# breuner/elbencho

Hardware: AMD Instinct MI355X
Metric: seq-read GiB/s into GPU HBM (higher is better)
Workload: dtype raw-bytes; 1 GPU; seqread; model=storage-benchmark seq-read into HBM, threads_per_gpu=16, block_size=4194304, iodepth=1, bench_dir=/dev/shm/elbencho_amd_bench, gpu_staged=True, mmap_zero_copy=True, dynamic_slice=True, verify_on_gpu=True, verify_salt=7, parallelism=single, device=AMD Radeon Graphics, device_numa_node=1

## Files before the change

elbencho_amd/csrc/engine.cpp:

```cpp

#include "engine.h"

#include <fcntl.h>
#include <linux/fs.h>
#include <pthread.h>
#include <sched.h>
#include <sys/ioctl.h>
#include <sys/mman.h>
#include <sys/stat.h>
#include <sys/types.h>
#include <unistd.h>

#include <algorithm>
#include <random>
#include <cerrno>
#include <cstdio>
#include <cstring>

#include "netbench.h"
#include "uring.h"

namespace eb {

static constexpr uint64_t INTERRUPT_CHECK_INTERVAL = 128;
// ... 477 lines not shown

    if (gpu && (fileOff % 8 == 0) && (len % 16 == 0)) {
        GpuVerifyResult r = gpu->verifyChecksumDev(slot, len, fileOff, (uint64_t)cfg.verifySalt);
        if (r.numMismatches)
            throw WorkerError("Data verification failed (GPU). First bad file offset: " +
                              std::to_string(r.firstBadFileOffset) +
                              "; mismatching 8-byte words: " + std::to_string(r.numMismatches));
        return;
    }

    uint64_t bad = verifyChecksumCPU(hostBufs[slot], len, fileOff, (uint64_t)cfg.verifySalt);
    if (bad != UINT64_MAX)
        throw WorkerError("Data verification failed. First bad file offset: " +
                          std::to_string(bad));
}


namespace {

struct FdGuard {
    std::vector<int> fds;
    ~FdGuard()
    {
        for (int fd : fds)
            if (fd >= 0) close(fd);
    }
};

struct MmapGuard {
    std::vector<std::pair<char*, uint64_t>> maps;

    void map(int fd, uint64_t len, bool writable, int madvFlags, const std::string& path)
    {
        int prot = writable ? (PROT_READ | PROT_WRITE) : PROT_READ;
        void* p = mmap(nullptr, len, prot, MAP_SHARED, fd, 0);
        if (p == MAP_FAILED)
            throw WorkerError("mmap failed. Path: " + path + "; SysErr: " + strerror(errno));
        if (madvFlags && madvise(p, len, madvFlags))
            throw WorkerError("madvise failed. Path: " + path);
        maps.emplace_back((char*)p, len);
    }

    char* base(uint64_t idx) const
    {
        return idx < maps.size() ? maps[idx].first : nullptr;
    }

    ~MmapGuard()
    {
        for (auto& [p, len] : maps) munmap(p, len);
    }
};

enum FadvBits {
    FADV_BIT_SEQ = 1,
    FADV_BIT_RAND = 2,
    FADV_BIT_WILLNEED = 4,
    FADV_BIT_DONTNEED = 8,
    FADV_BIT_NOREUSE = 16,
};

inline void applyFadvise(int fd, int bits, const std::string& path)
{
    if (!bits) return;
    struct { int bit; int advice; } table[] = {
        {FADV_BIT_SEQ, POSIX_FADV_SEQUENTIAL},   {FADV_BIT_RAND, POSIX_FADV_RANDOM},
        {FADV_BIT_WILLNEED, POSIX_FADV_WILLNEED}, {FADV_BIT_DONTNEED, POSIX_FADV_DONTNEED},
        {FADV_BIT_NOREUSE, POSIX_FADV_NOREUSE},
    };
    for (auto& e : table)
        if ((bits & e.bit) && posix_fadvise(fd, 0, 0, e.advice))
            throw WorkerError("posix_fadvise failed. Path: " + path);
}

}

void Worker::fileModeBlocks(bool isWrite)
{
    const auto& cfg = eng.cfg;
    if (cfg.ioDepth > 1) return fileModeBlocksUring(isWrite);
    if (cfg.useMmap && !cfg.gpuIDs.empty() && cfg.flockMode == 0 &&
        !(isWrite && (cfg.rwMixPct > 0 || cfg.rwMixThreads > 0)) && !cfg.verifyDirect &&
        cfg.pathType == PathType::FILE && !eng.opsLog.isEnabled())
        return fileModeBlocksGpuMmap(isWrite);

    const uint64_t fileSize = eng.effFileSize;
    const uint64_t bs = cfg.blockSize;
    const size_t numFiles = cfg.paths.size();
    const uint64_t numBlocksPerFile = (fileSize + bs - 1) / bs;
    const bool rwMixActive = isWrite && (cfg.rwMixPct > 0 || isDedicatedReader);

    FdGuard fg;
    MmapGuard mg;
    int rwFlags = isWrite
                      ? ((cfg.verifyDirect || rwMixActive || cfg.useMmap) ? O_RDWR : O_WRONLY)
                      : O_RDONLY;
    int openFlags = rwFlags | (cfg.directIO ? O_DIRECT : 0);
    if (isWrite && cfg.pathType == PathType::FILE) openFlags |= O_CREAT;
    for (const auto& p : cfg.paths) {
        int fd = open(p.c_str(), openFlags, 0644);
        if (fd < 0) throwErrno("open", p);
        fg.fds.push_back(fd);
        if (isWrite && cfg.pathType == PathType::FILE) {
            if (cfg.truncate && ftruncate(fd, 0)) throwErrno("truncate", p);
            if ((cfg.truncToSize != UINT64_MAX || cfg.useMmap) && ftruncate(fd, fileSize))
                throwErrno("truncate-to-size", p);
            if (cfg.preallocFile && fallocate(fd, 0, 0, fileSize)) throwErrno("fallocate", p);
        }
        applyFadvise(fd, cfg.fadviseFlags, p);
        if (cfg.useMmap) mg.map(fd, fileSize, isWrite, cfg.madviseFlags, p);
    }

    const uint64_t mapBPF = (cfg.random || cfg.strided) ? (fileSize / bs) : numBlocksPerFile;
    const uint64_t virtFileLen = mapBPF * bs;

    auto mapBlock = [&](const BlockSpec& s, uint64_t& fileIdx, uint64_t& inFileOff,
                        uint64_t& ioLen) -> bool {
        if (!virtFileLen) return false;
        fileIdx = s.offset / virtFileLen;
        if (fileIdx >= numFiles) return false;
        inFileOff = s.offset - fileIdx * virtFileLen;
        if (inFileOff >= fileSize) return false;
        ioLen = std::min(s.len, fileSize - inFileOff);
        return true;
    };

    std::unique_ptr<OffsetGen> gen;
    if (cfg.random || cfg.strided) {
        uint64_t numBlocksTotal = mapBPF * numFiles;
        uint64_t rangeLen = bs * (numBlocksTotal / cfg.numDataSetThreads);
        uint64_t rangeOff = (uint64_t)globalRank * rangeLen;
        if (cfg.strided) {
            gen = std::make_unique<OffsetGenStrided>(bs, globalRank, cfg.numDataSetThreads);
            gen->reset(0, bs * numBlocksTotal);
        } else {
            gen = makeOffsetGen(rangeOff, rangeLen);
        }
    } else {
        uint64_t myStart, myLen;
        fairShareSlice(virtFileLen * numFiles, myStart, myLen);
        if (!myLen) return;
        gen = makeOffsetGen(myStart, myLen);
    }

    static const bool pipelineDisabled = [] {
        const char* v = getenv("EB_GPU_PIPELINE");
        return v && v[0] == '0';
    }();
    const bool gpuPipelined = gpu && !pipelineDisabled && cfg.ioDepth == 1 &&
                              !cfg.useMmap && cfg.flockMode == 0 &&
                              !rwMixActive && !cfg.verifyDirect && hostBufs.size() >= 2 &&
                              !eng.opsLog.isEnabled();
    if (gpuPipelined) {
        constexpr uint64_t VERIFY_FETCH_INTERVAL = 64;
        const bool doVerify = cfg.verifySalt >= 0;
        const bool lat = cfg.measureLat;
        const int nSlots = (int)hostBufs.size();
        std::vector<char> slotBusy(nSlots, 0);
        uint64_t sinceFetch = 0;
        BlockSpec spec;
        uint64_t opCount = 0;

        auto fetchVerify = [&]() {
            GpuVerifyResult r = gpu->fetchVerifyResult();
            if (r.numMismatches)
                throw WorkerError(
                    "Data verification failed (GPU). First bad file offset: " +
                    std::to_string(r.firstBadFileOffset) + "; mismatching 8-byte words: " +
                    std::to_string(r.numMismatches));
        };

        if (isWrite) {
            int slot = 0;
            bool havePrev = false;
            int prevSlot = 0;
            uint64_t prevFileIdx = 0, prevInFileOff = 0, prevIoLen = 0;

            for (;;) {
                bool haveCur = false;
                uint64_t fileIdx = 0, inFileOff = 0, ioLen = 0;
                while (gen->next(spec)) {
                    if (mapBlock(spec, fileIdx, inFileOff, ioLen)) {
                        haveCur = true;
                        break;
                    }
                }

                if (haveCur) {
                    if ((opCount++ % INTERRUPT_CHECK_INTERVAL) == 0) checkInterrupt();
                    rateLimiter.wait(ioLen);
                    if (slotBusy[slot]) gpu->waitSlotEvent(slot);
                    preWriteFill(slot, ioLen, inFileOff);
                    if (lat) gpu->recordTimedStart(slot);
                    gpu->copyD2HAsync(slot, ioLen);
                    if (lat) gpu->recordTimedEnd(slot);
                    gpu->recordSlotEvent(slot);
                    slotBusy[slot] = 1;
                }

                if (havePrev) {
                    gpu->waitSlotEvent(prevSlot);
                    uint64_t copyUs = (lat && gpu->timedPairActive(prevSlot))
                                          ? gpu->timedElapsedUSec(prevSlot) : 0;
                    auto t0 = lat ? Clock::now() : Clock::time_point();
                    ssize_t res = pwrite(fg.fds[prevFileIdx], hostBufs[prevSlot],
                                         prevIoLen, prevInFileOff);
                    if (res != (ssize_t)prevIoLen) throwErrno("write", cfg.paths[prevFileIdx]);
                    if (lat)
                        addIoLat(copyUs + (uint64_t)std::chrono::duration_cast<
                            std::chrono::microseconds>(Clock::now() - t0).count());
                    liveOps.bytes.fetch_add(prevIoLen, std::memory_order_relaxed);
                    liveOps.iops.fetch_add(1, std::memory_order_relaxed);
                }

                if (!haveCur) break;
                havePrev = true;
                prevSlot = slot;
                prevFileIdx = fileIdx;
                prevInFileOff = inFileOff;
                prevIoLen = ioLen;
                slot = (slot + 1) % nSlots;
            }
            if (cfg.fsyncPerFile)
                for (size_t i = 0; i < fg.fds.size(); i++)
                    if (fsync(fg.fds[i])) throwErrno("fsync", cfg.paths[i]);
        } else if (!doVerify && gpuBatchSlots(cfg.blockSize) >= 2 && nSlots >= 4) {
            const int batch = gpuBatchSlots(cfg.blockSize);
            int half = 0;
            bool halfBusy[2] = {false, false};
            std::vector<uint64_t> blkUs[2];
            int halfCount[2] = {0, 0};
            if (lat) {
                blkUs[0].resize(batch);
                blkUs[1].resize(batch);
            }

            auto collectHalfLat = [&](int h) {
                if (!lat || !halfCount[h]) return;
                int b = h * batch;
                if (!gpu->timedPairActive(b)) return;
                uint64_t share = gpu->timedElapsedUSec(b) / (uint64_t)halfCount[h];
                for (int i = 0; i < halfCount[h]; i++)
                    addIoLat(blkUs[h][i] + share);
                halfCount[h] = 0;
            };

            int filled = 0;
            int base = 0;
            while (gen->next(spec)) {
                uint64_t fileIdx, inFileOff, ioLen;
                if (!mapBlock(spec, fileIdx, inFileOff, ioLen)) continue;

                if (filled == 0) {
                    if ((opCount++ % 4) == 0) checkInterrupt();
                    base = half * batch;
                    if (halfBusy[half]) {
                        gpu->waitSlotEvent(base);
                        collectHalfLat(half);
                    }
                }

                rateLimiter.wait(ioLen);
                auto t0 = lat ? Clock::now() : Clock::time_point();
                ssize_t res = pread(fg.fds[fileIdx], hostBufs[base + filled], ioLen,
                                    inFileOff);
                if (res != (ssize_t)ioLen) throwErrno("read", cfg.paths[fileIdx]);
                if (lat)
                    blkUs[half][filled] = (uint64_t)std::chrono::duration_cast<
                        std::chrono::microseconds>(Clock::now() - t0).count();
                liveOps.bytes.fetch_add(ioLen, std::memory_order_relaxed);
                liveOps.iops.fetch_add(1, std::memory_order_relaxed);
                filled++;

                if (filled == batch) {
                    if (lat) {
                        halfCount[half] = batch;
                        gpu->recordTimedStart(base);
                    }
                    gpu->copyH2DRangeAsync(base, batch);
                    if (lat) gpu->recordTimedEnd(base);
                    gpu->recordSlotEvent(base);
                    halfBusy[half] = true;
                    half ^= 1;
                    filled = 0;
                }
            }
            if (filled) {
                int b = half * batch;
                if (lat) {
                    halfCount[half] = filled;
                    gpu->recordTimedStart(b);
                }
                gpu->copyH2DRangeAsync(b, filled);
                if (lat) gpu->recordTimedEnd(b);
            }
            if (lat) {
                gpu->syncStream();
                collectHalfLat(0);
                collectHalfLat(1);
            }
        } else {
            int slot = 0;
            std::vector<uint64_t> preadUs(lat ? nSlots : 0, 0);
            while (gen->next(spec)) {
                if ((opCount++ % INTERRUPT_CHECK_INTERVAL) == 0) checkInterrupt();

                uint64_t fileIdx, inFileOff, ioLen;
                if (!mapBlock(spec, fileIdx, inFileOff, ioLen)) continue;

                rateLimiter.wait(ioLen);
                if (slotBusy[slot]) gpu->waitSlotEvent(slot);
                if (lat && gpu->timedPairActive(slot))
                    addIoLat(preadUs[slot] + gpu->timedElapsedUSec(slot));

                auto t0 = lat ? Clock::now() : Clock::time_point();
                ssize_t res = pread(fg.fds[fileIdx], hostBufs[slot], ioLen, inFileOff);
                if (res != (ssize_t)ioLen) throwErrno("read", cfg.paths[fileIdx]);
                if (lat) {
                    preadUs[slot] = (uint64_t)std::chrono::duration_cast<
                        std::chrono::microseconds>(Clock::now() - t0).count();
                    gpu->recordTimedStart(slot);
                }

                gpu->copyH2DAsync(slot, ioLen);
                if (lat) gpu->recordTimedEnd(slot);
                if (doVerify) {
                    if ((inFileOff % 8 == 0) && (ioLen % 16 == 0)) {
                        gpu->verifyChecksumDevAsync(slot, ioLen, inFileOff,
                                                    (uint64_t)cfg.verifySalt);
                        if (++sinceFetch >= VERIFY_FETCH_INTERVAL) {
                            fetchVerify();
                            sinceFetch = 0;
                        }
                    } else {
                        uint64_t bad = verifyChecksumCPU(hostBufs[slot], ioLen, inFileOff,
                                                         (uint64_t)cfg.verifySalt);
                        if (bad != UINT64_MAX)
                            throw WorkerError(
                                "Data verification failed. First bad file offset: " +
                                std::to_string(bad));
                    }
                }
                gpu->recordSlotEvent(slot);
                slotBusy[slot] = 1;

                liveOps.bytes.fetch_add(ioLen, std::memory_order_relaxed);
                liveOps.iops.fetch_add(1, std::memory_order_relaxed);
                slot = (slot + 1) % nSlots;
            }
            if (doVerify) fetchVerify();
            if (lat) {
                gpu->syncStream();
                for (int s = 0; s < nSlots; s++)
                    if (gpu->timedPairActive(s))
                        addIoLat(preadUs[s] + gpu->timedElapsedUSec(s));
            }
        }

        gpu->syncStream();
        return;
    }

    const bool lat = cfg.measureLat;
    BlockSpec spec;
    uint64_t opCount = 0;

    while (gen->next(spec)) {
        if ((opCount++ % INTERRUPT_CHECK_INTERVAL) == 0) checkInterrupt();

        uint64_t fileIdx, inFileOff, ioLen;
        if (!mapBlock(spec, fileIdx, inFileOff, ioLen)) continue;

        bool mixRead = rwMixActive &&
                       (isDedicatedReader ||
                        (cfg.rwMixThreads == 0 && rwMixDecideRead()));
        bool blockWrite = isWrite && !mixRead;

        if (rwMixActive && rwBalancerActive()) rwBalanceWait(mixRead, ioLen);

        auto t0 = lat ? Clock::now() : Clock::time_point();

        ssize_t res = blockIO(blockWrite, fg.fds[fileIdx], 0, ioLen, inFileOff,
                              mg.base(fileIdx), &cfg.paths[fileIdx]);
        if (res < 0)
            throwErrno(blockWrite ? "write" : "read", cfg.paths[fileIdx]);
        if ((uint64_t)res != ioLen)
            throw WorkerError(std::string("unexpected short ") + (blockWrite ? "write" : "read") +
                              ". Path: " + cfg.paths[fileIdx] +
                              "; expected: " + std::to_string(ioLen) +
                              "; got: " + std::to_string(res) +
                              (mixRead ? "; Hint: rwmix reads need a pre-written file." : ""));

        if (lat)
            addIoLat((uint64_t)std::chrono::duration_cast<std::chrono::microseconds>(
                Clock::now() - t0).count(), mixRead);

        AtomicLiveOps& ops = mixRead ? liveOpsReadMix : liveOps;
        ops.bytes.fetch_add(ioLen, std::memory_order_relaxed);
        ops.iops.fetch_add(1, std::memory_order_relaxed);
        if (rwMixActive && rwBalancerActive()) rwBalanceAccount(mixRead, ioLen);
    }

    if (isWrite && cfg.fsyncPerFile)
        for (size_t i = 0; i < fg.fds.size(); i++)
            if (fsync(fg.fds[i])) throwErrno("fsync", cfg.paths[i]);
}

void Worker::fileModeBlocksGpuMmap(bool isWrite)
{
    const auto& cfg = eng.cfg;
    const uint64_t fileSize = eng.effFileSize;
    const uint64_t bs = cfg.blockSize;
    const size_t numFiles = cfg.paths.size();
    const uint64_t numBlocksPerFile = (fileSize + bs - 1) / bs;
    const bool doVerify = cfg.verifySalt >= 0;
    const bool lat = cfg.measureLat;

    std::vector<char*> bases(numFiles);
    for (size_t i = 0; i < numFiles; i++)
        bases[i] = eng.getMappedReg(cfg.paths[i], fileSize, isWrite).base;

    const uint64_t mapBPF = (cfg.random || cfg.strided) ? (fileSize / bs) : numBlocksPerFile;
    const uint64_t virtFileLen = mapBPF * bs;

    const bool dynamic = cfg.dynamicSlice && !cfg.random && !cfg.strided &&
                         !cfg.backward && cfg.numThreads == cfg.numDataSetThreads;

    std::unique_ptr<OffsetGen> gen;
    if (dynamic) {
    } else if (cfg.random || cfg.strided) {
        uint64_t numBlocksTotal = mapBPF * numFiles;
        uint64_t rangeLen = bs * (numBlocksTotal / cfg.numDataSetThreads);
        uint64_t rangeOff = (uint64_t)globalRank * rangeLen;
        if (cfg.strided) {
            gen = std::make_unique<OffsetGenStrided>(bs, globalRank, cfg.numDataSetThreads);
            gen->reset(0, bs * numBlocksTotal);
        } else {
            gen = makeOffsetGen(rangeOff, rangeLen);
        }
    } else {
        uint64_t myStart, myLen;
        fairShareSlice(virtFileLen * numFiles, myStart, myLen);
        if (!myLen) return;
        gen = makeOffsetGen(myStart, myLen);
    }

    const int nSlots = (int)hostBufs.size();
    constexpr uint64_t VERIFY_FETCH_INTERVAL = 64;
    uint64_t sinceFetch = 0;
    BlockSpec spec;
    uint64_t opCount = 0;
    int slot = 0;

    auto fetchVerify = [&]() {
        GpuVerifyResult r = gpu->fetchVerifyResult();
        if (r.numMismatches)
            throw WorkerError("Data verification failed (GPU). First bad file offset: " +
                              std::to_string(r.firstBadFileOffset) +
                              "; mismatching 8-byte words: " +
                              std::to_string(r.numMismatches));
    };

    const uint64_t totalBlocks = numBlocksPerFile * numFiles;

    auto nextBlock = [&](uint64_t& fileIdx, uint64_t& inFileOff,
                         uint64_t& ioLen) -> bool {
        if (dynamic) {
            for (;;) {
                uint64_t b = eng.dynCursor.fetch_add(1, std::memory_order_relaxed);
                if (b >= totalBlocks) return false;
                fileIdx = b / numBlocksPerFile;
                inFileOff = (b % numBlocksPerFile) * bs;
                if (inFileOff >= fileSize) continue;
                ioLen = std::min(bs, fileSize - inFileOff);
                return true;
            }
        }
        while (gen->next(spec)) {
            if (!virtFileLen) return false;
            fileIdx = spec.offset / virtFileLen;
            if (fileIdx >= numFiles) continue;
            inFileOff = spec.offset - fileIdx * virtFileLen;
            if (inFileOff >= fileSize) continue;
            ioLen = std::min(spec.len, fileSize - inFileOff);
            return true;
        }
        return false;
    };

    uint64_t fileIdx, inFileOff, ioLen;
    while (nextBlock(fileIdx, inFileOff, ioLen)) {
        if ((opCount++ % INTERRUPT_CHECK_INTERVAL) == 0) checkInterrupt();

        rateLimiter.wait(ioLen);

        if (lat && gpu->timedPairActive(slot))
            addIoLat(gpu->timedElapsedUSec(slot));

        if (isWrite) {
            preWriteFill(slot, ioLen, inFileOff);
            if (lat) gpu->recordTimedStart(slot);
            gpu->copyToHostAsync(slot, bases[fileIdx] + inFileOff, ioLen);
            if (lat) gpu->recordTimedEnd(slot);
        } else {
            if (lat) gpu->recordTimedStart(slot);
            gpu->copyFromHostAsync(slot, bases[fileIdx] + inFileOff, ioLen);
            if (lat) gpu->recordTimedEnd(slot);
            if (doVerify && (inFileOff % 8 == 0) && (ioLen % 16 == 0)) {
                gpu->verifyChecksumDevAsync(slot, ioLen, inFileOff,
                                            (uint64_t)cfg.verifySalt);
                if (++sinceFetch >= VERIFY_FETCH_INTERVAL) {
                    fetchVerify();
                    sinceFetch = 0;
                }
            } else if (doVerify) {
                uint64_t bad = verifyChecksumCPU(bases[fileIdx] + inFileOff, ioLen,
                                                 inFileOff, (uint64_t)cfg.verifySalt);
                if (bad != UINT64_MAX)
                    throw WorkerError("Data verification failed. First bad file offset: " +
                                      std::to_string(bad));
            }
        }

        liveOps.bytes.fetch_add(ioLen, std::memory_order_relaxed);
        liveOps.iops.fetch_add(1, std::memory_order_relaxed);
        slot = (slot + 1) % nSlots;

        if ((opCount & 127) == 0) gpu->syncStream();
    }

    gpu->syncStream();
    if (lat)
        for (int s = 0; s < nSlots; s++)
            if (gpu->timedPairActive(s)) addIoLat(gpu->timedElapsedUSec(s));
    if (doVerify && !isWrite) fetchVerify();
}

void Worker::fileModeBlocksUring(bool isWrite)
{
    const auto& cfg = eng.cfg;
    const uint64_t fileSize = eng.effFileSize;
    const uint64_t bs = cfg.blockSize;
    const size_t numFiles = cfg.paths.size();
    const uint64_t numBlocksPerFile = (fileSize + bs - 1) / bs;
    const int depth = cfg.ioDepth;
    const bool lat = cfg.measureLat;

    const bool rwMixActive = isWrite && (cfg.rwMixPct > 0 || isDedicatedReader);

    FdGuard fg;
    int rwFlags = isWrite ? ((cfg.verifyDirect || rwMixActive) ? O_RDWR : O_WRONLY) : O_RDONLY;
    int openFlags = rwFlags | (cfg.directIO ? O_DIRECT : 0);
    if (isWrite && cfg.pathType == PathType::FILE) openFlags |= O_CREAT;
    for (const auto& p : cfg.paths) {
        int fd = open(p.c_str(), openFlags, 0644);
        if (fd < 0) throwErrno("open", p);
        fg.fds.push_back(fd);
        if (isWrite && cfg.pathType == PathType::FILE) {
            if (cfg.truncate && ftruncate(fd, 0)) throwErrno("truncate", p);
            if (cfg.truncToSize != UINT64_MAX && ftruncate(fd, fileSize))
                throwErrno("truncate-to-size", p);
            if (cfg.preallocFile && fallocate(fd, 0, 0, fileSize)) throwErrno("fallocate", p);
        }
        applyFadvise(fd, cfg.fadviseFlags, p);
    }

    const uint64_t mapBPF = (cfg.random || cfg.strided) ? (fileSize / bs) : numBlocksPerFile;
    const uint64_t virtFileLen = mapBPF * bs;

    auto mapBlock = [&](const BlockSpec& s, uint64_t& fileIdx, uint64_t& inFileOff,
                        uint64_t& ioLen) -> bool {
        if (!virtFileLen) return false;
        fileIdx = s.offset / virtFileLen;
        if (fileIdx >= numFiles) return false;
        inFileOff = s.offset - fileIdx * virtFileLen;
        if (inFileOff >= fileSize) return false;
        ioLen = std::min(s.len, fileSize - inFileOff);
        return true;
    };

    std::unique_ptr<OffsetGen> gen;
    if (cfg.random || cfg.strided) {
        uint64_t numBlocksTotal = mapBPF * numFiles;
        uint64_t rangeLen = bs * (numBlocksTotal / cfg.numDataSetThreads);
        uint64_t rangeOff = (uint64_t)globalRank * rangeLen;
        if (cfg.strided) {
            gen = std::make_unique<OffsetGenStrided>(bs, globalRank, cfg.numDataSetThreads);
            gen->reset(0, bs * numBlocksTotal);
        } else {
            gen = makeOffsetGen(rangeOff, rangeLen);
        }
    } else {
        uint64_t myStart, myLen;
        fairShareSlice(virtFileLen * numFiles, myStart, myLen);
        if (!myLen) return;
        gen = makeOffsetGen(myStart, myLen);
    }

    IoUring ring;
    ring.init(depth);

    if (!getenv("EB_URING_NOFIXED")) {
        std::vector<struct iovec> iovs(depth);
        for (int s = 0; s < depth; s++)
            iovs[s] = {hostBufs[s], (size_t)bs};
        ring.registerBuffers(iovs.data(), depth);
        ring.registerFiles(fg.fds.data(), (unsigned)fg.fds.size());
    }

    const int gpuBatch = gpu ? gpuBatchSlots(bs) : 1;
    const bool batchedRead = gpu && !isWrite && cfg.verifySalt < 0 &&
                             gpuBatch >= 2 && depth >= 4 &&
                             getenv("EB_GPU_URING_BATCH");
    if (getenv("EB_DEBUG_PATH"))
        fprintf(stderr, "[eb] uring path: gpu=%d batchedRead=%d batch=%d depth=%d\n",
                gpu ? 1 : 0, (int)batchedRead, gpuBatch, depth);
    if (batchedRead) {
        const int halfSize = std::min(depth / 2, 64);
        struct Op {
            uint64_t off = 0, len = 0;
            Clock::time_point start;
            int fileIdx = 0;
        };
        std::vector<Op> ops(2 * halfSize);
        std::vector<IoUring::Completion> bcomps(depth);
        int submitted[2] = {0, 0}, done[2] = {0, 0};
        bool exhausted2 = false;
        BlockSpec bspec;

        auto fillHalf = [&](int h) -> int {
            int base = h * halfSize;
            int n = 0;
            while (n < halfSize && !exhausted2) {
                uint64_t fileIdx = 0, inFileOff = 0, ioLen = 0;
                for (;;) {
                    if (!gen->next(bspec)) { exhausted2 = true; break; }
                    if (mapBlock(bspec, fileIdx, inFileOff, ioLen)) break;
                }
                if (exhausted2) break;
                rateLimiter.wait(ioLen);
                int slot = base + n;
                ops[slot] = {inFileOff, ioLen,
                             lat ? Clock::now() : Clock::time_point(), (int)fileIdx};
                if (eng.opsLog.isEnabled())
                    eng.opsLog.log(globalRank, "uring_read", cfg.paths[fileIdx],
                                   inFileOff, ioLen, true, false);
                int rfd = ring.hasFixedFiles() ? (int)fileIdx : fg.fds[fileIdx];
                while (!ring.prep(false, rfd, hostBufs[slot], ioLen, inFileOff,
                                  (uint64_t)slot,
                                  ring.hasFixedBuffers() ? slot : -1,
                                  ring.hasFixedFiles())) {
                    ring.submitAndWait(0);
                    checkInterrupt();
                }
                n++;
            }
            submitted[h] = n;
            done[h] = 0;
            return n;
        };

        int inFlightB = fillHalf(0) + fillHalf(1);
        uint64_t opCountB = 0;
        while (inFlightB > 0) {
            checkInterrupt();
            ring.submitAndWait(1, 250);
            unsigned n = ring.reap(bcomps.data(), depth);
            for (unsigned i = 0; i < n; i++) {
                int slot = (int)bcomps[i].userData;
                const Op& op = ops[slot];
                if (eng.opsLog.isEnabled())
                    eng.opsLog.log(globalRank, "uring_read", cfg.paths[op.fileIdx],
                                   op.off, op.len, false, bcomps[i].res < 0);
                if (bcomps[i].res < 0)
                    throw WorkerError(std::string("async read failed. Path: ") +
                                      cfg.paths[op.fileIdx] + "; SysErr: " +
                                      strerror(-bcomps[i].res));
                if ((uint64_t)bcomps[i].res != op.len)
                    throw WorkerError("unexpected short async read. Path: " +
                                      cfg.paths[op.fileIdx]);
                if (lat)
                    addIoLat((uint64_t)std::chrono::duration_cast<
                        std::chrono::microseconds>(Clock::now() - op.start).count());
                liveOps.bytes.fetch_add(op.len, std::memory_order_relaxed);
                liveOps.iops.fetch_add(1, std::memory_order_relaxed);
                done[slot / halfSize]++;
                inFlightB--;
                if ((opCountB++ % INTERRUPT_CHECK_INTERVAL) == 0) checkInterrupt();
// ... 1716 lines not shown
```

elbencho_amd/csrc/gpu.h:

```cpp

#pragma once

#include <cstdint>
#include <string>

namespace eb {

struct GpuVerifyResult {
    uint64_t numMismatches;
    uint64_t firstBadFileOffset;
};

void gpuHostRegister(void* ptr, uint64_t len);
bool gpuHostRegisterTry(void* ptr, uint64_t len);
void gpuHostUnregister(void* ptr);

class GpuCtx;

int gpuDeviceCount();

double gpuVerifyBenchGBs(uint64_t len, int iters, bool lds, int dev);

std::string gpuProbeError();

std::string gpuDeviceName(int deviceId);

int gpuNumaNode(int deviceId);

class GpuCtx {
public:
    GpuCtx(int deviceId, int numSlots, uint64_t bufSize, bool pinnedHostBufs);
    ~GpuCtx();
    GpuCtx(const GpuCtx&) = delete;
    GpuCtx& operator=(const GpuCtx&) = delete;

    int deviceId() const { return devId; }
    char* hostBuf(int slot) const;
    uint64_t bufSize() const { return slotSize; }
    int numSlots() const { return slots; }

    void bindThread();

    void copyFromHostAsync(int slot, const void* src, uint64_t len);
    void copyToHostAsync(int slot, void* dst, uint64_t len);
    void copyH2DAsync(int slot, uint64_t len);
    void copyH2DRangeAsync(int firstSlot, int count);
    void copyD2HAsync(int slot, uint64_t len);
    void syncStream();

    void recordSlotEvent(int slot);
    void waitSlotEvent(int slot);

    void recordTimedStart(int slot);
    void recordTimedEnd(int slot);
    bool timedPairActive(int slot) const;
    uint64_t timedElapsedUSec(int slot);

    void verifyChecksumDevAsync(int slot, uint64_t len, uint64_t fileOff, uint64_t salt);
    GpuVerifyResult fetchVerifyResult();


    void fillRandDev(int slot, uint64_t len, uint64_t seed, bool fastAlgo = false);

    void fillChecksumDev(int slot, uint64_t len, uint64_t fileOff, uint64_t salt);

    GpuVerifyResult verifyChecksumDev(int slot, uint64_t len, uint64_t fileOff, uint64_t salt);

    void blockVarRefillDev(int slot, uint64_t len, uint64_t refillLen, uint64_t seed,
                           bool fastAlgo = false);

private:
    struct Impl;
    Impl* impl;
    int devId;
    uint64_t slotSize;
    int slots;
};

}
```

elbencho_amd/csrc/gpu_kernels.hip:

```cpp

#include <hip/hip_runtime.h>

#include <cstdio>
#include <map>
#include <mutex>
#include <stdexcept>
#include <string>
#include <vector>

#include "gpu.h"

namespace eb {

#define HIP_CHECK(cmd)                                                                 \
    do {                                                                               \
        hipError_t e = (cmd);                                                          \
        if (e != hipSuccess)                                                           \
            throw std::runtime_error(std::string("HIP error: ") + hipGetErrorString(e) \
                                     + " at " __FILE__ ":" + std::to_string(__LINE__)); \
    } while (0)


__device__ __forceinline__ uint64_t d_splitmix64(uint64_t& state)
{
    uint64_t z = (state += 0x9E3779B97F4A7C15ULL);
    z = (z ^ (z >> 30)) * 0xBF58476D1CE4E5B9ULL;
    z = (z ^ (z >> 27)) * 0x94D049BB133111EBULL;
    return z ^ (z >> 31);
}

__device__ __forceinline__ uint64_t d_rotl64(uint64_t x, int k)
{
    return (x << k) | (x >> (64 - k));
}

struct Xoshiro256pp {
    uint64_t s0, s1, s2, s3;

    __device__ void seed(uint64_t seedVal)
    {
        uint64_t sm = seedVal;
        s0 = d_splitmix64(sm);
        s1 = d_splitmix64(sm);
        s2 = d_splitmix64(sm);
        s3 = d_splitmix64(sm);
    }

    __device__ __forceinline__ uint64_t next()
    {
        const uint64_t result = d_rotl64(s0 + s3, 23) + s0;
        const uint64_t t = s1 << 17;
        s2 ^= s0;
        s3 ^= s1;
        s1 ^= s2;
        s0 ^= s3;
        s2 ^= t;
        s3 = d_rotl64(s3, 45);
        return result;
    }
};


constexpr int FILL_U64S_PER_STEP = 8;

__global__ __launch_bounds__(256) void ebFillRandKernel(ulonglong2* __restrict__ buf,
                                                        uint64_t nVec2,
                                                        uint64_t seed)
{
    uint64_t tid = (uint64_t)blockIdx.x * blockDim.x + threadIdx.x;
    uint64_t stride = (uint64_t)gridDim.x * blockDim.x;

    Xoshiro256pp rngA, rngB;
    rngA.seed(seed ^ (tid * 0xA24BAED4963EE407ULL));
    rngB.seed(seed ^ (tid * 0xA24BAED4963EE407ULL) ^ 0x9E6D62D06F6A9A9BULL);

    constexpr int VEC_PER_STEP = FILL_U64S_PER_STEP / 2;
    for (uint64_t base = tid * VEC_PER_STEP; base < nVec2; base += stride * VEC_PER_STEP) {
#pragma unroll
        for (int v = 0; v < VEC_PER_STEP; v++) {
            uint64_t idx = base + v;
            if (idx < nVec2) {
                ulonglong2 val;
                val.x = rngA.next();
                val.y = rngB.next();
                buf[idx] = val;
            }
        }
    }
}

__global__ __launch_bounds__(256) void ebFillFastKernel(ulonglong2* __restrict__ buf,
                                                        uint64_t nVec2,
                                                        uint64_t seed)
{
    uint64_t tid = (uint64_t)blockIdx.x * blockDim.x + threadIdx.x;
    uint64_t stride = (uint64_t)gridDim.x * blockDim.x;
    for (uint64_t idx = tid; idx < nVec2; idx += stride) {
        uint64_t s0 = seed + idx * 2 * 0x9E3779B97F4A7C15ULL;
        uint64_t s1 = s0 + 0x9E3779B97F4A7C15ULL;
        ulonglong2 val;
        uint64_t z = s0;
        z = (z ^ (z >> 30)) * 0xBF58476D1CE4E5B9ULL;
        z = (z ^ (z >> 27)) * 0x94D049BB133111EBULL;
        val.x = z ^ (z >> 31);
        z = s1;
        z = (z ^ (z >> 30)) * 0xBF58476D1CE4E5B9ULL;
        z = (z ^ (z >> 27)) * 0x94D049BB133111EBULL;
        val.y = z ^ (z >> 31);
        buf[idx] = val;
    }
}

__global__ __launch_bounds__(256) void ebBlockVarFastKernel(ulonglong2* __restrict__ buf,
                                                            uint64_t nVec2,
                                                            uint64_t refillVec2,
                                                            uint64_t seed,
                                                            uint64_t fillConst)
{
    uint64_t tid = (uint64_t)blockIdx.x * blockDim.x + threadIdx.x;
    uint64_t stride = (uint64_t)gridDim.x * blockDim.x;
    for (uint64_t idx = tid; idx < nVec2; idx += stride) {
        ulonglong2 val;
        if (idx < refillVec2) {
            uint64_t s0 = seed + idx * 2 * 0x9E3779B97F4A7C15ULL;
            uint64_t z = s0;
            z = (z ^ (z >> 30)) * 0xBF58476D1CE4E5B9ULL;
            z = (z ^ (z >> 27)) * 0x94D049BB133111EBULL;
            val.x = z ^ (z >> 31);
            z = s0 + 0x9E3779B97F4A7C15ULL;
            z = (z ^ (z >> 30)) * 0xBF58476D1CE4E5B9ULL;
            z = (z ^ (z >> 27)) * 0x94D049BB133111EBULL;
            val.y = z ^ (z >> 31);
        } else {
            val.x = fillConst;
            val.y = fillConst;
        }
        buf[idx] = val;
    }
}

__global__ __launch_bounds__(256) void ebFillChecksumKernel(uint64_t* __restrict__ buf,
                                                            uint64_t n64,
                                                            uint64_t fileOff,
                                                            uint64_t salt)
{
    uint64_t tid = (uint64_t)blockIdx.x * blockDim.x + threadIdx.x;
    uint64_t stride = (uint64_t)gridDim.x * blockDim.x;
    uint64_t nVec2 = n64 / 2;
    ulonglong2* __restrict__ v = (ulonglong2*)buf;
    for (uint64_t i = tid; i < nVec2; i += stride) {
        ulonglong2 val;
        val.x = fileOff + i * 16 + salt;
        val.y = fileOff + i * 16 + 8 + salt;
        v[i] = val;
    }
    if (tid == 0 && (n64 & 1))
        buf[n64 - 1] = fileOff + (n64 - 1) * 8 + salt;
}

__global__ __launch_bounds__(256) void ebVerifyChecksumKernel(const ulonglong2* __restrict__ buf,
                                                              uint64_t nVec2,
                                                              uint64_t fileOff,
                                                              uint64_t salt,
                                                              unsigned long long* __restrict__ out)
{
    uint64_t tid = (uint64_t)blockIdx.x * blockDim.x + threadIdx.x;
    uint64_t stride = (uint64_t)gridDim.x * blockDim.x;

    unsigned long long localBad = 0;
    unsigned long long localFirst = ~0ULL;

    for (uint64_t i = tid; i < nVec2; i += stride) {
        ulonglong2 v = buf[i];
        uint64_t off0 = fileOff + i * 16;
        uint64_t exp0 = off0 + salt;
        uint64_t exp1 = off0 + 8 + salt;
        if (v.x != exp0) {
            localBad++;
            if (off0 < localFirst) localFirst = off0;
        }
        if (v.y != exp1) {
            localBad++;
            if (off0 + 8 < localFirst) localFirst = off0 + 8;
        }
    }

#pragma unroll
    for (int delta = 32; delta > 0; delta >>= 1) {
        localBad += __shfl_down(localBad, delta, 64);
        unsigned long long other = __shfl_down(localFirst, delta, 64);
        if (other < localFirst) localFirst = other;
    }

    if ((threadIdx.x & 63) == 0 && localBad) {
        atomicAdd(&out[0], localBad);
        atomicMin(&out[1], localFirst);
    }
}

__global__ __launch_bounds__(256) void ebVerifyChecksumLdsKernel(
    const ulonglong2* __restrict__ buf, uint64_t nVec2, uint64_t fileOff,
    uint64_t salt, unsigned long long* __restrict__ out)
{
    constexpr int VPT = 4;
    __shared__ ulonglong2 lds[256 * VPT];
    __shared__ unsigned long long blkBad, blkFirst;
    if (threadIdx.x == 0) {
        blkBad = 0;
        blkFirst = ~0ULL;
    }
    __syncthreads();

    unsigned long long localBad = 0, localFirst = ~0ULL;
    const uint64_t tileElems = (uint64_t)blockDim.x * VPT;

    for (uint64_t tileBase = (uint64_t)blockIdx.x * tileElems; tileBase < nVec2;
         tileBase += (uint64_t)gridDim.x * tileElems) {
#pragma unroll
        for (int v = 0; v < VPT; v++) {
            uint64_t idx = tileBase + (uint64_t)v * blockDim.x + threadIdx.x;
            if (idx < nVec2) lds[v * blockDim.x + threadIdx.x] = buf[idx];
        }
        __syncthreads();
#pragma unroll
        for (int v = 0; v < VPT; v++) {
            uint64_t idx = tileBase + (uint64_t)v * blockDim.x + threadIdx.x;
            if (idx >= nVec2) continue;
            ulonglong2 val = lds[v * blockDim.x + threadIdx.x];
            uint64_t off0 = fileOff + idx * 16;
            if (val.x != off0 + salt) {
                localBad++;
                if (off0 < localFirst) localFirst = off0;
            }
            if (val.y != off0 + 8 + salt) {
                localBad++;
                if (off0 + 8 < localFirst) localFirst = off0 + 8;
            }
        }
        __syncthreads();
    }

#pragma unroll
    for (int delta = 32; delta > 0; delta >>= 1) {
        localBad += __shfl_down(localBad, delta, 64);
        unsigned long long other = __shfl_down(localFirst, delta, 64);
        if (other < localFirst) localFirst = other;
    }
    if ((threadIdx.x & 63) == 0 && localBad) {
        atomicAdd(&blkBad, localBad);
        atomicMin(&blkFirst, localFirst);
    }
    __syncthreads();
    if (threadIdx.x == 0 && blkBad) {
        atomicAdd(&out[0], blkBad);
        atomicMin(&out[1], blkFirst);
    }
}

__global__ __launch_bounds__(256) void ebBlockVarKernel(ulonglong2* __restrict__ buf,
                                                        uint64_t nVec2,
                                                        uint64_t refillVec2,
                                                        uint64_t seed,
                                                        uint64_t fillConst)
{
    uint64_t tid = (uint64_t)blockIdx.x * blockDim.x + threadIdx.x;
    uint64_t stride = (uint64_t)gridDim.x * blockDim.x;

    Xoshiro256pp rngA, rngB;
    rngA.seed(seed ^ (tid * 0xA24BAED4963EE407ULL));
    rngB.seed(seed ^ (tid * 0xA24BAED4963EE407ULL) ^ 0x9E6D62D06F6A9A9BULL);

    constexpr int VEC_PER_STEP = FILL_U64S_PER_STEP / 2;
    for (uint64_t base = tid * VEC_PER_STEP; base < nVec2; base += stride * VEC_PER_STEP) {
#pragma unroll
        for (int v = 0; v < VEC_PER_STEP; v++) {
            uint64_t idx = base + v;
            if (idx < nVec2) {
                ulonglong2 val;
                if (idx < refillVec2) {
                    val.x = rngA.next();
                    val.y = rngB.next();
                } else {
                    val.x = fillConst;
                    val.y = fillConst;
                }
                buf[idx] = val;
            }
        }
    }
}


double gpuVerifyBenchGBs(uint64_t len, int iters, bool lds, int dev);

bool gpuHostRegisterTry(void* ptr, uint64_t len)
{
    return hipHostRegister(ptr, len, hipHostRegisterDefault) == hipSuccess;
}

void gpuHostRegister(void* ptr, uint64_t len)
{
    HIP_CHECK(hipHostRegister(ptr, len, hipHostRegisterDefault));
}

void gpuHostUnregister(void* ptr) { (void)hipHostUnregister(ptr); }

int gpuDeviceCount()
{
    int n = 0;
    hipError_t e = hipGetDeviceCount(&n);
    if (e != hipSuccess) return 0;
    return n;
}

std::string gpuProbeError()
{
    int n = 0;
    hipError_t e = hipGetDeviceCount(&n);
    if (e != hipSuccess) return hipGetErrorString(e);
    return "ok: " + std::to_string(n) + " device(s)";
}

std::string gpuDeviceName(int deviceId)
{
    hipDeviceProp_t prop;
    if (hipGetDeviceProperties(&prop, deviceId) != hipSuccess) return "";
    return prop.name;
}

int gpuNumaNode(int deviceId)
{
    char busId[32] = {0};
    if (hipDeviceGetPCIBusId(busId, sizeof(busId), deviceId) != hipSuccess)
        return -1;
    for (char* c = busId; *c; ++c) *c = (char)tolower(*c);
    std::string path = std::string("/sys/bus/pci/devices/") + busId + "/numa_node";
    FILE* f = fopen(path.c_str(), "r");
    if (!f) return -1;
    int node = -1;
    if (fscanf(f, "%d", &node) != 1) node = -1;
    fclose(f);
    return node;
}

static dim3 gridForBytes(uint64_t workItems)
{
    uint64_t blocks = (workItems + 255) / 256;
    if (blocks > 4096) blocks = 4096;
    if (blocks == 0) blocks = 1;
    return dim3((uint32_t)blocks);
}

static hipStream_t sharedStream(int devId, int& poolSizeOut)
{
    static std::mutex mtx;
    static std::map<int, std::vector<hipStream_t>> pools;
    static std::map<int, int> next;
    static const int poolSize = [] {
        const char* v = getenv("EB_GPU_SHARED_STREAMS");
        int n = v ? atoi(v) : 8;
        return (n >= 1 && n <= 64) ? n : 0;
    }();

    poolSizeOut = poolSize;
    if (!poolSize) return nullptr;

    std::lock_guard<std::mutex> lk(mtx);
    auto& pool = pools[devId];
    if (pool.empty()) {
        pool.resize(poolSize);
        for (int i = 0; i < poolSize; i++)
            HIP_CHECK(hipStreamCreateWithFlags(&pool[i], hipStreamNonBlocking));
    }
    return pool[next[devId]++ % poolSize];
}

struct GpuCtx::Impl {
    hipStream_t stream = nullptr;
    bool ownStream = true;
    char* devBase = nullptr;
    char* hostBase = nullptr;
    uint64_t slotStride = 0;
    std::vector<char*> devBufs;
    std::vector<char*> hostBufs;
    std::vector<hipEvent_t> slotEvents;
    std::vector<hipEvent_t> timedStart, timedEnd;
    std::vector<char> timedActive;
    bool hostPinned = false;
    unsigned long long* verifyOutDev = nullptr;
    unsigned long long* verifyOutHost = nullptr;
    uint64_t fillCallCounter = 0;
    bool verifyDirty = false;
};

GpuCtx::GpuCtx(int deviceId, int numSlots, uint64_t bufSize, bool pinnedHostBufs)
    : impl(new Impl), devId(deviceId), slotSize(bufSize), slots(numSlots)
{
    HIP_CHECK(hipSetDevice(deviceId));
    int poolSize = 0;
    hipStream_t shared = sharedStream(deviceId, poolSize);
    if (shared) {
        impl->stream = shared;
        impl->ownStream = false;
    } else {
        HIP_CHECK(hipStreamCreateWithFlags(&impl->stream, hipStreamNonBlocking));
    }

    impl->hostPinned = pinnedHostBufs;
    impl->devBufs.resize(numSlots, nullptr);
    impl->hostBufs.resize(numSlots, nullptr);

    impl->slotStride = (bufSize + 4095) & ~4095ULL;
    HIP_CHECK(hipMalloc(&impl->devBase, impl->slotStride * numSlots));
    if (pinnedHostBufs) {
        static const unsigned hostFlags = [] {
            const char* v = getenv("EB_GPU_HOSTALLOC");
            return (v && v[0] == 'n') ? hipHostMallocNonCoherent : hipHostMallocDefault;
        }();
        HIP_CHECK(hipHostMalloc(&impl->hostBase, impl->slotStride * numSlots, hostFlags));
    } else {
        if (posix_memalign((void**)&impl->hostBase, 4096, impl->slotStride * numSlots))
            throw std::runtime_error("host buffer alloc failed");
    }
    for (int i = 0; i < numSlots; i++) {
        impl->devBufs[i] = impl->devBase + (uint64_t)i * impl->slotStride;
        impl->hostBufs[i] = impl->hostBase + (uint64_t)i * impl->slotStride;
    }

    impl->slotEvents.resize(numSlots, nullptr);
    static const bool evBlock = [] {
        const char* v = getenv("EB_GPU_EVBLOCK");
        return v && v[0] == '1';
    }();
    unsigned evFlags = hipEventDisableTiming | (evBlock ? hipEventBlockingSync : 0);
    for (int i = 0; i < numSlots; i++)
        HIP_CHECK(hipEventCreateWithFlags(&impl->slotEvents[i], evFlags));

    HIP_CHECK(hipMalloc(&impl->verifyOutDev, 2 * sizeof(unsigned long long)));
    HIP_CHECK(hipHostMalloc(&impl->verifyOutHost, 2 * sizeof(unsigned long long),
                            hipHostMallocDefault));

    impl->verifyOutHost[0] = 0;
    impl->verifyOutHost[1] = ~0ULL;
    HIP_CHECK(hipMemcpy(impl->verifyOutDev, impl->verifyOutHost,
                        2 * sizeof(unsigned long long), hipMemcpyHostToDevice));
}

GpuCtx::~GpuCtx()
{
    (void)hipSetDevice(devId);
    if (impl->devBase) (void)hipFree(impl->devBase);
    if (impl->hostBase) {
        if (impl->hostPinned)
            (void)hipHostFree(impl->hostBase);
        else
            free(impl->hostBase);
    }
    for (auto e : impl->slotEvents)
        if (e) (void)hipEventDestroy(e);
    for (auto e : impl->timedStart)
        if (e) (void)hipEventDestroy(e);
    for (auto e : impl->timedEnd)
        if (e) (void)hipEventDestroy(e);
    if (impl->verifyOutDev) (void)hipFree(impl->verifyOutDev);
    if (impl->verifyOutHost) (void)hipHostFree(impl->verifyOutHost);
    if (impl->stream && impl->ownStream) (void)hipStreamDestroy(impl->stream);
    delete impl;
}

char* GpuCtx::hostBuf(int slot) const { return impl->hostBufs[slot]; }

void GpuCtx::bindThread() { HIP_CHECK(hipSetDevice(devId)); }

void GpuCtx::copyFromHostAsync(int slot, const void* src, uint64_t len)
{
    HIP_CHECK(hipMemcpyAsync(impl->devBufs[slot], src, len, hipMemcpyHostToDevice,
                             impl->stream));
}

void GpuCtx::copyToHostAsync(int slot, void* dst, uint64_t len)
{
    HIP_CHECK(hipMemcpyAsync(dst, impl->devBufs[slot], len, hipMemcpyDeviceToHost,
                             impl->stream));
}

void GpuCtx::copyH2DAsync(int slot, uint64_t len)
{
    HIP_CHECK(hipMemcpyAsync(impl->devBufs[slot], impl->hostBufs[slot], len,
                             hipMemcpyHostToDevice, impl->stream));
}

void GpuCtx::copyH2DRangeAsync(int firstSlot, int count)
{
    HIP_CHECK(hipMemcpyAsync(impl->devBufs[firstSlot], impl->hostBufs[firstSlot],
                             impl->slotStride * count, hipMemcpyHostToDevice,
                             impl->stream));
}

void GpuCtx::copyD2HAsync(int slot, uint64_t len)
{
    HIP_CHECK(hipMemcpyAsync(impl->hostBufs[slot], impl->devBufs[slot], len,
                             hipMemcpyDeviceToHost, impl->stream));
}

void GpuCtx::syncStream() { HIP_CHECK(hipStreamSynchronize(impl->stream)); }

void GpuCtx::recordSlotEvent(int slot)
{
    HIP_CHECK(hipEventRecord(impl->slotEvents[slot], impl->stream));
}

void GpuCtx::waitSlotEvent(int slot)
{
    HIP_CHECK(hipEventSynchronize(impl->slotEvents[slot]));
}


void GpuCtx::recordTimedStart(int slot)
{
    if (impl->timedStart.empty()) {
        impl->timedStart.resize(slots, nullptr);
        impl->timedEnd.resize(slots, nullptr);
        impl->timedActive.assign(slots, 0);
        for (int i = 0; i < slots; i++) {
            HIP_CHECK(hipEventCreateWithFlags(&impl->timedStart[i], hipEventDefault));
            HIP_CHECK(hipEventCreateWithFlags(&impl->timedEnd[i], hipEventDefault));
        }
    }
    HIP_CHECK(hipEventRecord(impl->timedStart[slot], impl->stream));
}

void GpuCtx::recordTimedEnd(int slot)
{
    HIP_CHECK(hipEventRecord(impl->timedEnd[slot], impl->stream));
    impl->timedActive[slot] = 1;
}

bool GpuCtx::timedPairActive(int slot) const
{
    return !impl->timedActive.empty() && impl->timedActive[slot];
}

uint64_t GpuCtx::timedElapsedUSec(int slot)
{
    HIP_CHECK(hipEventSynchronize(impl->timedEnd[slot]));
    float ms = 0;
    HIP_CHECK(hipEventElapsedTime(&ms, impl->timedStart[slot], impl->timedEnd[slot]));
    impl->timedActive[slot] = 0;
    return (uint64_t)(ms * 1000.0f);
}

void GpuCtx::verifyChecksumDevAsync(int slot, uint64_t len, uint64_t fileOff, uint64_t salt)
{
    uint64_t nVec2 = len / 16;
    if (!nVec2) return;
    dim3 grid = gridForBytes(nVec2);
    hipLaunchKernelGGL(ebVerifyChecksumKernel, grid, dim3(256), 0, impl->stream,
                       (const ulonglong2*)impl->devBufs[slot], nVec2, fileOff, salt,
                       impl->verifyOutDev);
    HIP_CHECK(hipGetLastError());
    impl->verifyDirty = true;
}

GpuVerifyResult GpuCtx::fetchVerifyResult()
{
    if (!impl->verifyDirty) return GpuVerifyResult{0, ~0ULL};
    HIP_CHECK(hipMemcpyAsync(impl->verifyOutHost, impl->verifyOutDev,
                             2 * sizeof(unsigned long long), hipMemcpyDeviceToHost,
                             impl->stream));
    HIP_CHECK(hipStreamSynchronize(impl->stream));
    GpuVerifyResult r{impl->verifyOutHost[0], impl->verifyOutHost[1]};
    impl->verifyOutHost[0] = 0;
    impl->verifyOutHost[1] = ~0ULL;
    HIP_CHECK(hipMemcpyAsync(impl->verifyOutDev, impl->verifyOutHost,
                             2 * sizeof(unsigned long long), hipMemcpyHostToDevice,
                             impl->stream));
    HIP_CHECK(hipStreamSynchronize(impl->stream));
    impl->verifyDirty = false;
    return r;
}

void GpuCtx::fillRandDev(int slot, uint64_t len, uint64_t seed, bool fastAlgo)
{
    uint64_t nVec2 = len / 16;
    uint64_t seq = ++impl->fillCallCounter;
    if (nVec2) {
        if (fastAlgo) {
            dim3 grid = gridForBytes(nVec2);
            hipLaunchKernelGGL(ebFillFastKernel, grid, dim3(256), 0, impl->stream,
                               (ulonglong2*)impl->devBufs[slot], nVec2,
                               seed + seq * 0x9E3779B9ULL);
        } else {
            dim3 grid = gridForBytes(nVec2 / (FILL_U64S_PER_STEP / 2));
            hipLaunchKernelGGL(ebFillRandKernel, grid, dim3(256), 0, impl->stream,
                               (ulonglong2*)impl->devBufs[slot], nVec2,
                               seed + seq * 0x9E3779B9ULL);
        }
        HIP_CHECK(hipGetLastError());
    }
}

void GpuCtx::fillChecksumDev(int slot, uint64_t len, uint64_t fileOff, uint64_t salt)
{
    uint64_t n64 = len / 8;
    if (!n64) return;
    dim3 grid = gridForBytes(n64);
    hipLaunchKernelGGL(ebFillChecksumKernel, grid, dim3(256), 0, impl->stream,
                       (uint64_t*)impl->devBufs[slot], n64, fileOff, salt);
    HIP_CHECK(hipGetLastError());
}

GpuVerifyResult GpuCtx::verifyChecksumDev(int slot, uint64_t len, uint64_t fileOff, uint64_t salt)
{
    verifyChecksumDevAsync(slot, len, fileOff, salt);
    return fetchVerifyResult();
}

void GpuCtx::blockVarRefillDev(int slot, uint64_t len, uint64_t refillLen, uint64_t seed,
                               bool fastAlgo)
{
    uint64_t nVec2 = len / 16;
    if (!nVec2) return;
    uint64_t refillVec2 = refillLen / 16;
    uint64_t seq = ++impl->fillCallCounter;
    uint64_t sm = seed + seq;
    uint64_t z = (sm += 0x9E3779B97F4A7C15ULL);
    z = (z ^ (z >> 30)) * 0xBF58476D1CE4E5B9ULL;
    z = (z ^ (z >> 27)) * 0x94D049BB133111EBULL;
    uint64_t fillConst = z ^ (z >> 31);

    if (fastAlgo) {
        dim3 grid = gridForBytes(nVec2);
        hipLaunchKernelGGL(ebBlockVarFastKernel, grid, dim3(256), 0, impl->stream,
                           (ulonglong2*)impl->devBufs[slot], nVec2, refillVec2,
                           seed + seq * 0x9E3779B9ULL, fillConst);
    } else {
        dim3 grid = gridForBytes(nVec2 / (FILL_U64S_PER_STEP / 2));
        hipLaunchKernelGGL(ebBlockVarKernel, grid, dim3(256), 0, impl->stream,
                           (ulonglong2*)impl->devBufs[slot], nVec2, refillVec2,
                           seed + seq * 0x9E3779B9ULL, fillConst);
    }
    HIP_CHECK(hipGetLastError());
}

double gpuVerifyBenchGBs(uint64_t len, int iters, bool lds, int dev)
{
    HIP_CHECK(hipSetDevice(dev));
    const uint64_t nVec2 = len / 16;
    ulonglong2* buf = nullptr;
    unsigned long long* out = nullptr;
    HIP_CHECK(hipMalloc(&buf, len));
    HIP_CHECK(hipMalloc(&out, 2 * sizeof(unsigned long long)));
    HIP_CHECK(hipMemset(out, 0, 2 * sizeof(unsigned long long)));

    hipStream_t s;
    HIP_CHECK(hipStreamCreateWithFlags(&s, hipStreamNonBlocking));
    dim3 grid = gridForBytes(nVec2);

    hipLaunchKernelGGL(ebFillChecksumKernel, gridForBytes(len / 8), dim3(256), 0, s,
                       (uint64_t*)buf, len / 8, 0, 7);

    auto launch = [&] {
        if (lds)
            hipLaunchKernelGGL(ebVerifyChecksumLdsKernel, grid, dim3(256), 0, s,
                               buf, nVec2, 0, 7, out);
        else
            hipLaunchKernelGGL(ebVerifyChecksumKernel, grid, dim3(256), 0, s,
                               buf, nVec2, 0, 7, out);
    };

    launch();
    launch();
    HIP_CHECK(hipStreamSynchronize(s));

    hipEvent_t e0, e1;
    HIP_CHECK(hipEventCreate(&e0));
    HIP_CHECK(hipEventCreate(&e1));
    HIP_CHECK(hipEventRecord(e0, s));
    for (int i = 0; i < iters; i++) launch();
    HIP_CHECK(hipEventRecord(e1, s));
    HIP_CHECK(hipEventSynchronize(e1));
    float ms = 0;
    HIP_CHECK(hipEventElapsedTime(&ms, e0, e1));

    (void)hipEventDestroy(e0);
    (void)hipEventDestroy(e1);
    (void)hipStreamDestroy(s);
    (void)hipFree(buf);
    (void)hipFree(out);

    return (double)len * iters / (ms / 1000.0) / 1e9;
}

}
```

Before: 52.04 GiB/s.

## Signal GPU verify mismatches via pinned host flag instead of periodic stream syncs

```diff
diff --git a/elbencho_amd/csrc/engine.cpp b/elbencho_amd/csrc/engine.cpp
--- a/elbencho_amd/csrc/engine.cpp
+++ b/elbencho_amd/csrc/engine.cpp
@@ -653,17 +653,16 @@
                               !rwMixActive && !cfg.verifyDirect && hostBufs.size() >= 2 &&
                               !eng.opsLog.isEnabled();
     if (gpuPipelined) {
-        constexpr uint64_t VERIFY_FETCH_INTERVAL = 64;
         const bool doVerify = cfg.verifySalt >= 0;
         const bool lat = cfg.measureLat;
         const int nSlots = (int)hostBufs.size();
         std::vector<char> slotBusy(nSlots, 0);
-        uint64_t sinceFetch = 0;
+        bool ownWorkDone = false;
         BlockSpec spec;
         uint64_t opCount = 0;
 
-        auto fetchVerify = [&]() {
-            GpuVerifyResult r = gpu->fetchVerifyResult();
+        auto checkVerify = [&]() {
+            GpuVerifyResult r = gpu->checkVerifyResult();
             if (r.numMismatches)
                 throw WorkerError(
                     "Data verification failed (GPU). First bad file offset: " +
@@ -813,6 +812,7 @@
                 if (slotBusy[slot]) gpu->waitSlotEvent(slot);
                 if (lat && gpu->timedPairActive(slot))
                     addIoLat(preadUs[slot] + gpu->timedElapsedUSec(slot));
+                if (doVerify && gpu->peekVerifyFlag()) checkVerify();
 
                 auto t0 = lat ? Clock::now() : Clock::time_point();
                 ssize_t res = pread(fg.fds[fileIdx], hostBufs[slot], ioLen, inFileOff);
@@ -829,10 +829,6 @@
                     if ((inFileOff % 8 == 0) && (ioLen % 16 == 0)) {
                         gpu->verifyChecksumDevAsync(slot, ioLen, inFileOff,
                                                     (uint64_t)cfg.verifySalt);
-                        if (++sinceFetch >= VERIFY_FETCH_INTERVAL) {
-                            fetchVerify();
-                            sinceFetch = 0;
-                        }
                     } else {
                         uint64_t bad = verifyChecksumCPU(hostBufs[slot], ioLen, inFileOff,
                                                          (uint64_t)cfg.verifySalt);
@@ -849,16 +845,17 @@
                 liveOps.iops.fetch_add(1, std::memory_order_relaxed);
                 slot = (slot + 1) % nSlots;
             }
-            if (doVerify) fetchVerify();
-            if (lat) {
-                gpu->syncStream();
+            for (int s = 0; s < nSlots; s++)
+                if (slotBusy[s]) gpu->waitSlotEvent(s);
+            if (lat)
                 for (int s = 0; s < nSlots; s++)
                     if (gpu->timedPairActive(s))
                         addIoLat(preadUs[s] + gpu->timedElapsedUSec(s));
-            }
-        }
-
-        gpu->syncStream();
+            if (doVerify) checkVerify();
+            ownWorkDone = true;
+        }
+
+        if (!ownWorkDone) gpu->syncStream();
         return;
     }
 
@@ -947,14 +944,14 @@
     }
 
     const int nSlots = (int)hostBufs.size();
-    constexpr uint64_t VERIFY_FETCH_INTERVAL = 64;
-    uint64_t sinceFetch = 0;
+    std::vector<char> slotBusy(nSlots, 0);
     BlockSpec spec;
     uint64_t opCount = 0;
     int slot = 0;
-
-    auto fetchVerify = [&]() {
-        GpuVerifyResult r = gpu->fetchVerifyResult();
+    int lastSlot = -1;
+
+    auto checkVerify = [&]() {
+        GpuVerifyResult r = gpu->checkVerifyResult();
         if (r.numMismatches)
             throw WorkerError("Data verification failed (GPU). First bad file offset: " +
                               std::to_string(r.firstBadFileOffset) +
@@ -997,6 +994,10 @@
 
         if (lat && gpu->timedPairActive(slot))
             addIoLat(gpu->timedElapsedUSec(slot));
+        else if (slotBusy[slot])
+            gpu->waitSlotEvent(slot);
+
+        if (doVerify && !isWrite && gpu->peekVerifyFlag()) checkVerify();
 
         if (isWrite) {
             preWriteFill(slot, ioLen, inFileOff);
@@ -1010,10 +1011,6 @@
             if (doVerify && (inFileOff % 8 == 0) && (ioLen % 16 == 0)) {
                 gpu->verifyChecksumDevAsync(slot, ioLen, inFileOff,
                                             (uint64_t)cfg.verifySalt);
-                if (++sinceFetch >= VERIFY_FETCH_INTERVAL) {
-                    fetchVerify();
-                    sinceFetch = 0;
-                }
             } else if (doVerify) {
                 uint64_t bad = verifyChecksumCPU(bases[fileIdx] + inFileOff, ioLen,
                                                  inFileOff, (uint64_t)cfg.verifySalt);
@@ -1023,18 +1020,29 @@
             }
         }
 
+        if (!lat && !isWrite) {
+            gpu->recordSlotEvent(slot);
+            slotBusy[slot] = 1;
+        }
+
         liveOps.bytes.fetch_add(ioLen, std::memory_order_relaxed);
         liveOps.iops.fetch_add(1, std::memory_order_relaxed);
+        lastSlot = slot;
         slot = (slot + 1) % nSlots;
 
-        if ((opCount & 127) == 0) gpu->syncStream();
-    }
-
-    gpu->syncStream();
+        if (isWrite && (opCount & 127) == 0) gpu->syncStream();
+    }
+
+    if (isWrite) {
+        gpu->syncStream();
+    } else if (lastSlot >= 0) {
+        if (lat) gpu->recordSlotEvent(lastSlot);
+        gpu->waitSlotEvent(lastSlot);
+    }
     if (lat)
         for (int s = 0; s < nSlots; s++)
             if (gpu->timedPairActive(s)) addIoLat(gpu->timedElapsedUSec(s));
-    if (doVerify && !isWrite) fetchVerify();
+    if (doVerify && !isWrite) checkVerify();
 }
 
 void Worker::fileModeBlocksUring(bool isWrite)
diff --git a/elbencho_amd/csrc/gpu.h b/elbencho_amd/csrc/gpu.h
--- a/elbencho_amd/csrc/gpu.h
+++ b/elbencho_amd/csrc/gpu.h
@@ -57,6 +57,8 @@
     uint64_t timedElapsedUSec(int slot);
 
     void verifyChecksumDevAsync(int slot, uint64_t len, uint64_t fileOff, uint64_t salt);
+    bool peekVerifyFlag() const;
+    GpuVerifyResult checkVerifyResult();
     GpuVerifyResult fetchVerifyResult();
 
 
diff --git a/elbencho_amd/csrc/gpu_kernels.hip b/elbencho_amd/csrc/gpu_kernels.hip
--- a/elbencho_amd/csrc/gpu_kernels.hip
+++ b/elbencho_amd/csrc/gpu_kernels.hip
@@ -162,7 +162,8 @@
                                                               uint64_t nVec2,
                                                               uint64_t fileOff,
                                                               uint64_t salt,
-                                                              unsigned long long* __restrict__ out)
+                                                              unsigned long long* __restrict__ out,
+                                                              unsigned int* __restrict__ hostFlag)
 {
     uint64_t tid = (uint64_t)blockIdx.x * blockDim.x + threadIdx.x;
     uint64_t stride = (uint64_t)gridDim.x * blockDim.x;
@@ -195,6 +196,10 @@
     if ((threadIdx.x & 63) == 0 && localBad) {
         atomicAdd(&out[0], localBad);
         atomicMin(&out[1], localFirst);
+        if (hostFlag) {
+            *(volatile unsigned int*)hostFlag = 1u;
+            __threadfence_system();
+        }
     }
 }
 
@@ -389,6 +394,8 @@
     bool hostPinned = false;
     unsigned long long* verifyOutDev = nullptr;
     unsigned long long* verifyOutHost = nullptr;
+    volatile unsigned int* verifyFlagHost = nullptr;
+    unsigned int* verifyFlagDev = nullptr;
     uint64_t fillCallCounter = 0;
     bool verifyDirty = false;
 };
@@ -437,8 +444,15 @@
         HIP_CHECK(hipEventCreateWithFlags(&impl->slotEvents[i], evFlags));
 
     HIP_CHECK(hipMalloc(&impl->verifyOutDev, 2 * sizeof(unsigned long long)));
-    HIP_CHECK(hipHostMalloc(&impl->verifyOutHost, 2 * sizeof(unsigned long long),
+    constexpr size_t VERIFY_HOST_WORDS = 16, VERIFY_FLAG_WORD = 8;
+    HIP_CHECK(hipHostMalloc(&impl->verifyOutHost,
+                            VERIFY_HOST_WORDS * sizeof(unsigned long long),
                             hipHostMallocDefault));
+    impl->verifyFlagHost =
+        (volatile unsigned int*)&impl->verifyOutHost[VERIFY_FLAG_WORD];
+    *impl->verifyFlagHost = 0;
+    HIP_CHECK(hipHostGetDevicePointer((void**)&impl->verifyFlagDev,
+                                      (void*)impl->verifyFlagHost, 0));
 
     impl->verifyOutHost[0] = 0;
     impl->verifyOutHost[1] = ~0ULL;
@@ -557,9 +571,17 @@
     dim3 grid = gridForBytes(nVec2);
     hipLaunchKernelGGL(ebVerifyChecksumKernel, grid, dim3(256), 0, impl->stream,
                        (const ulonglong2*)impl->devBufs[slot], nVec2, fileOff, salt,
-                       impl->verifyOutDev);
+                       impl->verifyOutDev, impl->verifyFlagDev);
     HIP_CHECK(hipGetLastError());
     impl->verifyDirty = true;
+}
+
+bool GpuCtx::peekVerifyFlag() const { return *impl->verifyFlagHost != 0; }
+
+GpuVerifyResult GpuCtx::checkVerifyResult()
+{
+    if (!peekVerifyFlag()) return GpuVerifyResult{0, ~0ULL};
+    return fetchVerifyResult();
 }
 
 GpuVerifyResult GpuCtx::fetchVerifyResult()
@@ -576,6 +598,7 @@
                              2 * sizeof(unsigned long long), hipMemcpyHostToDevice,
                              impl->stream));
     HIP_CHECK(hipStreamSynchronize(impl->stream));
+    *impl->verifyFlagHost = 0;
     impl->verifyDirty = false;
     return r;
 }
@@ -666,7 +689,7 @@
                                buf, nVec2, 0, 7, out);
         else
             hipLaunchKernelGGL(ebVerifyChecksumKernel, grid, dim3(256), 0, s,
-                               buf, nVec2, 0, 7, out);
+                               buf, nVec2, 0, 7, out, (unsigned int*)nullptr);
     };
 
     launch();
```

Result: no change. 52.04 GiB/s (-0.0%).
